# jason-huang03/SPH_Project

Hardware: AMD Instinct MI355X
Metric: particle-updates/sec (higher is better)
Workload: dtype f32

## Files before the change

### sph_project_amd/csrc/sph_device.hpp

```cpp
#pragma once
#include "sph_common.hpp"
#include <limits.h>

#ifndef SPH_FAST
#define SPH_FAST 0
#endif

__device__ __forceinline__ float fdiv(float a, float b) {
#if SPH_FAST
    return a * __builtin_amdgcn_rcpf(b);
#else
    return a / b;
#endif
}
__device__ __forceinline__ float fdiv2(float a, float b, float c) {
#if SPH_FAST
    return a * __builtin_amdgcn_rcpf(b * c);
#else
    return (a / b) / c;
#endif
}
__device__ __forceinline__ float fsqrt(float a) {
#if SPH_FAST
    return __builtin_amdgcn_sqrtf(a);
// ... 676 lines not shown
            const unsigned by = (cy > 0 ? 1u : 0u) | 2u | (cy < c.ny - 1 ? 4u : 0u);
            my_dom = (cx > 0 ? by : 0u) | (by << 3) | (cx < c.nx - 1 ? by << 6 : 0u);
        }
    }
    (&s_cnt[0][0])[tid] = 0;
    if (blk_flag) {
        const int anyf = __syncthreads_or((i < n && META_ACTIVE_FLUID(meta_i)) ? 1 : 0);
        if (tid == 0) blk_flag[blockIdx.x] = anyf ? 1 : 0;
    }
    unsigned long long peers = ~0ull;
#pragma unroll
    for (int bit = 0; bit < 6; ++bit) {
        const bool on = (key >> bit) & 1;
        const unsigned long long bal = __ballot(on);
        peers &= on ? bal : ~bal;
    }
    const unsigned long long below = (1ull << lane) - 1ull;
    const int rank_in_wave = __popcll(peers & below);
    __syncthreads();
    if (cellw && i < n) {
        const int e0 = (my_lin - s_c[0]) + my_dz0 + 1;
        cellw[i] = (unsigned)(e0 & 0xff) | ((unsigned)(my_dz + 1) << 8) | (my_dom << 11);
    }
    if ((peers & below) == 0ull) s_cnt[w][key] = __popcll(peers);
    if (tid < 9) {
        const int cfirst = s_c[0], clast = s_c[1];
        const int shift = (tid / 3 - 1) * c.ny * c.nz + (tid % 3 - 1) * c.nz;
        int lo = cfirst + shift - 1, hi = clast + shift + 1;
        int rs = 0, re = 0;
        if (clast >= cfirst && hi >= 0 && lo <= c.G - 1) {
            lo = lo < 0 ? 0 : lo;
            hi = hi > c.G - 1 ? c.G - 1 : hi;
            rs = cell_start[lo];
            re = cell_start[hi + 1];
        }
        int *h = blk_hdr + (size_t)blockIdx.x * BLK_HDR_INTS;
        if (tid == 0) { h[0] = cfirst; h[1] = clast; }
        h[2 + tid] = rs;
        h[11 + tid] = re - rs;
    }
    __syncthreads();
    if (perm) {
        const int tot = s_cnt[0][lane] + s_cnt[1][lane] + s_cnt[2][lane] + s_cnt[3][lane];
        const int incl = wave_incl_scan(tot);
        int dest = __shfl(incl - tot, key, 64) + rank_in_wave;
        for (int k = 0; k < w; ++k) dest += s_cnt[k][key];
        perm[i0 + dest] = (unsigned char)tid;
    }
}

__global__ void __launch_bounds__(256)
k_block_prep(const Consts c, const float4 *__restrict__ posv, const int *__restrict__ meta,
             const int *__restrict__ cell_start, int *__restrict__ blk_hdr, unsigned char *__restrict__ perm,
             int *__restrict__ blk_flag, const int *__restrict__ xidx, BlockPrepTables tabs, TilePlanOut plan, unsigned *__restrict__ cellw) {
    __shared__ int s_cnt[4][64];
    __shared__ int s_c[2];
    const int tid = threadIdx.x;
    const int i0 = blockIdx.x * 256;
    const int i = i0 + tid;
    const int n = live_n(c);
    if (plan.list_b && tid == 64 && i0 < n) {
        const int layer = c.ny * c.nz;
        const int r1 = plan.lo_layers > 0 ? cell_start[(plan.lo_layers < c.nx ? plan.lo_layers : c.nx) * layer] : 0;
        const int r2 = plan.hi_layers > 0 ? cell_start[(c.nx - plan.hi_layers > 0 ? c.nx - plan.hi_layers : 0) * layer] : n;
        const int nt = (n + 255) >> 8;
        int t1 = (r1 + 255) >> 8, t2 = r2 >> 8;
        if (t2 > nt) t2 = nt;
        if (t2 < t1) t2 = t1 = nt;
        const int t = (int)blockIdx.x, ni = t2 - t1;
        if (t < t1) plan.list_b[t] = t;
        else if (t >= t2) plan.list_b[t1 + (t - t2)] = t;
        else plan.list_i[t - t1] = t1 + xcd_remap(t - t1, ni);
        plan.cls[t] = (t < t1 || t >= t2) ? 1 : 0;
        if (t == 0) {
            plan.cnt[0] = nt - ni; plan.cnt[1] = ni;
            if (nt - ni > plan.bound_b && plan.status) atomicOr(plan.status, SLAB_ST_BOUND);
            if (plan.mirror_nb) *plan.mirror_nb = nt - ni;
        }
    }
    if (i0 >= n) {
        if (blk_flag && tid == 0) blk_flag[blockIdx.x] = 0;
        return;
    }
    float4 p = make_float4(0.f, 0.f, 0.f, 0.f);
    int meta_i = 0;
    if (i < n) {
        if (xidx) {
            const int x = xidx[i];
            const int kind = (int)(((unsigned)x) >> 28);
            if (kind >= 1 && kind <= 8) tabs.tab[kind - 1][x & 0x0fffffff] = i;
        }
        p = posv[i];
        if (blk_flag) meta_i = meta[i];
    }
    block_prep_tile(c, n, p, meta_i, cell_start, blk_hdr, perm, blk_flag, cellw, s_cnt, s_c);
}

__global__ void __launch_bounds__(256)
k_gather_prep(const Consts c, int n, const int *__restrict__ inv, SortArrays a, const int *__restrict__ cell_start,
              int *__restrict__ blk_hdr, unsigned char *__restrict__ perm, int *__restrict__ blk_flag, unsigned *__restrict__ cellw) {
    __shared__ int s_cnt[4][64];
    __shared__ int s_c[2];
    const int d = blockIdx.x * 256 + threadIdx.x;
    float4 p = make_float4(0.f, 0.f, 0.f, 0.f);
    int meta_i = 0;
    if (d < n) {
        const int i = inv[d];
        p = a.posv_in[i];
        meta_i = a.meta_in[i];
        a.posv_out[d] = p;
        a.velm_out[d] = a.velm_in[i];
        a.meta_out[d] = meta_i;
        a.pid_out[d] = a.pid_in[i];
        if (a.color_in) a.color_out[d] = a.color_in[i];
        if (a.rho_in) a.rho_out[d] = a.rho_in[i];
        if (a.orig_in) a.orig_out[d] = a.orig_in[i];
    }
    block_prep_tile(c, n, p, meta_i, cell_start, blk_hdr, perm, blk_flag, cellw, s_cnt, s_c);
}

__global__ void __launch_bounds__(256)
k_color_from_home(int n, const int *__restrict__ pid, const unsigned *__restrict__ home, unsigned *__restrict__ color) {
    const int i = blockIdx.x * 256 + threadIdx.x;
    if (i < n) color[i] = home[pid[i]];
}

__global__ void __launch_bounds__(256)
k_compact_blocks(const int *__restrict__ flag, int nb, int *__restrict__ list, int *__restrict__ count, volatile int *count_host) {
    __shared__ int s_w[4];
    const int per = (nb + 255) / 256;
    const int lo = threadIdx.x * per, hi = lo + per < nb ? lo + per : nb;
    int mine = 0;
    for (int b = lo; b < hi; ++b) mine += flag[b] ? 1 : 0;
    int tot;
    int at = block_excl_scan_256(mine, s_w, tot);
    for (int b = lo; b < hi; ++b) if (flag[b]) list[at++] = b;
    if (threadIdx.x == 0) { *count = tot; if (count_host) *count_host = tot; }
}

constexpr int SPH_NBR_LIGHT_CAP = 1280;
constexpr int SPH_NBR_HEAVY_BUDGET = 40960;
constexpr int SPH_NBR_MEDIUM_BYTES = 28;
constexpr int SPH_HEAVY_SB = 3;
constexpr int SPH_MEDIUM_SB = 3;
template <class P> constexpr int pass_slot_bytes() {
    return 16 + (P::HAS_B ? (int)sizeof(typename P::BT) : 0) + (PassC<P>::value ? (int)sizeof(typename PassC<P>::type) : 0);
}
template <class P, class = void> struct PassMediumOk { static constexpr bool value = false; };
template <class P> struct PassMediumOk<P, decltype((void)P::MEDIUM_OK)> { static constexpr bool value = P::MEDIUM_OK; };
template <class P> constexpr bool pass_is_medium() {
    return SPH_FAST && P::HAS_B && !pass_builds_masks<P>() &&
           (pass_slot_bytes<P>() <= SPH_NBR_MEDIUM_BYTES || (PassMediumOk<P>::value && pass_slot_bytes<P>() <= 32));
}
template <class P> constexpr int nbr_tile_cap() {
    const int per_slot = pass_slot_bytes<P>();
    const int budget = pass_is_medium<P>() ? 32768 : SPH_NBR_HEAVY_BUDGET;
    const int slots = (budget - 9 * NBR_CS_PITCH * 2 - 1536) / per_slot - NBR_PAD;
    return slots > SPH_NBR_LIGHT_CAP ? SPH_NBR_LIGHT_CAP : slots / 8 * 8;
}
__device__ __forceinline__ int run_of(int grouping, int g, int q) {
    const int i = g * 3 + q;
    return grouping ? (int)((0x861543720ull >> (4 * i)) & 15ull) : i;
}

template <int CAP>
__device__ __forceinline__ void nbr_plan(const int *__restrict__ hdr, int g, int qa, int fg, int (&rs_)[3], int (&ln_)[3], int (&lo_)[3],
                                         int &total, int &qb, unsigned &rm, bool &overflow, int grouping) {
    total = 0; qb = 3; rm = 7u; overflow = false;
#pragma unroll
    for (int q = 0; q < 3; ++q) {
        const int k = run_of(grouping, g, q);
        rs_[q] = hdr[2 + k];
        ln_[q] = hdr[11 + k] > 0 ? hdr[11 + k] : 0;
    }
    const int ulen = rs_[2] + ln_[2] - rs_[0];
    const bool chain = !grouping && ln_[0] > 0 && ln_[1] > 0 && ln_[2] > 0 && rs_[1] >= rs_[0] && rs_[1] <= rs_[0] + ln_[0] &&
                       rs_[2] >= rs_[1] && rs_[2] <= rs_[1] + ln_[1] && ulen >= ln_[2];
    if (qa == 0 && chain && ulen <= CAP && fg != 1 && fg != 5) {
        lo_[0] = lo_[1] = lo_[2] = -rs_[0];
        total = ulen;
    } else if (qa == 0 && ln_[0] + ln_[1] + ln_[2] <= CAP && fg != 1) {
        lo_[0] = -rs_[0]; lo_[1] = ln_[0] - rs_[1]; lo_[2] = ln_[0] + ln_[1] - rs_[2];
        total = ln_[0] + ln_[1] + ln_[2];
    } else {
        rm = 0u; qb = qa;
#pragma unroll
        for (int q = 0; q < 3; ++q) {
            lo_[q] = INT_MIN;
            if (q >= qa && q == qb && !overflow) {
                if (fg != 1 && total + ln_[q] <= CAP) { lo_[q] = total - rs_[q]; total += ln_[q]; qb = q + 1; rm |= 1u << q; }
                else if (q == qa) { overflow = true; qb = q + 1; rm |= 1u << q; }
            }
        }
    }
}
#ifdef SPH_TIMELINE
#define NBR_STAMP(k) do { if (timeline && threadIdx.x == 0) timeline[(size_t)blockIdx.x * 16 + (k)] = __builtin_readcyclecounter(); } while (0)
#else
#define NBR_STAMP(k) do { } while (0)
#endif
template <class P, int MASKMODE> constexpr int nbr_lds_bytes() {
    return (nbr_tile_cap<P>() + ((MASKMODE == 2 || pass_reuses_masks<P>()) ? 0 : NBR_PAD)) * (16 + (P::HAS_B ? (int)sizeof(typename P::BT) : 0) + (PassC<P>::value ? (int)sizeof(typename PassC<P>::type) : 0)) + 9 * NBR_CS_PITCH * 2 + 64;
}
constexpr int SPH_NBR_WAVES_LIGHT = SPH_FAST ? 6 : 4;
constexpr int SPH_NBR_WAVES_HEAVY = SPH_FAST ? 4 : 3;
template <class P, class = void> struct PassMaxWaves { static constexpr int value = 8; };
template <class P> struct PassMaxWaves<P, decltype((void)P::MAX_WAVES)> { static constexpr int value = P::MAX_WAVES; };
template <class P, int MASKMODE> constexpr int nbr_waves_per_simd() {
    const int w = P::HAS_B ? (pass_is_medium<P>() ? 5 : SPH_NBR_WAVES_HEAVY) : (sizeof(typename P::Own) <= 8 ? SPH_NBR_WAVES_LIGHT : 4);
    return w < PassMaxWaves<P>::value ? w : PassMaxWaves<P>::value;
}
__device__ __forceinline__ int split_lo(int ny, int y) { return ny == 3 ? y : (y == 0 ? 0 : 2); }
__device__ __forceinline__ int split_hi(int ny, int y) { return ny == 3 ? y + 1 : (y == 0 ? 2 : 3); }
template <class P, int MASKMODE>
__global__ void __launch_bounds__(P::BLOCK, (nbr_waves_per_simd<P, MASKMODE>()))
k_nbr_pass(const Consts c, const int *__restrict__ cell_start, const P p, DevScalars *__restrict__ scal,
           int nblocks, unsigned *__restrict__ nbr_mask, unsigned *__restrict__ nbr_mask_hi, int mask_stride,
           const int *__restrict__ blk_hdr, const unsigned char *__restrict__ lane_perm,
           unsigned long long *__restrict__ timeline, const int *__restrict__ stop_flag,
           const int *__restrict__ blk_list, const int *__restrict__ blk_count, const unsigned char *__restrict__ tile_skip) {
    const int stop_now = stop_flag ? *stop_flag : 0;
    const int list_len = blk_list ? *blk_count : INT_MAX;
    const int b_listed = blk_list ? blk_list[blockIdx.x] : 0;
    if (stop_now) return;
    if ((int)blockIdx.x >= list_len) {
        if constexpr (PassPrologue<P>::value) { if (blockIdx.x == 0 && blockIdx.y == 0) p.prologue(scal); }
        return;
    }
    constexpr int BLOCK = P::BLOCK;
    constexpr int CAP = nbr_tile_cap<P>();
    constexpr int NS = (CAP + BLOCK - 1) / BLOCK;
    constexpr int GROUPS = 3, RPG = 3;
    static_assert(P::GROUPS == 3 && BLOCK == 256, "lane permutation is stored as one byte per particle");
    typedef typename P::Own Own;
    typedef typename P::BT BT;
    constexpr int PAD = (MASKMODE == 2 || pass_reuses_masks<P>()) ? 0 : NBR_PAD;
    __shared__ float2 sT[2 * (CAP + PAD)];
    float2 *const sXY = sT;
    float2 *const sZW = sT + (CAP + PAD);
    constexpr int ZW_OFF = (CAP + PAD) * 8;
    __shared__ BT sB[P::HAS_B ? CAP + PAD : 1];
    __shared__ typename PassC<P>::type sC[PassC<P>::value ? CAP + PAD : 1];
    __shared__ unsigned short s_cs[9][NBR_CS_PITCH];
    __shared__ int s_loff[9];

    const int tid = threadIdx.x;
    NBR_STAMP(0);
    const int b = blk_list ? b_listed : xcd_remap(blockIdx.x, nblocks, c.xcd_chunk);
    const int i0 = b * BLOCK;
    const int who_early = lane_perm ? (int)lane_perm[i0 + tid] : tid;
    const int *hdr = blk_hdr + (size_t)b * BLK_HDR_INTS;
    const int cfirst = hdr[0], clast = hdr[1];
    const int skip_tile = tile_skip ? (int)tile_skip[b] : 0;
    const int n_live = live_n(c);
    if constexpr (PassWrench<P>::value) wrench_init_all(p.pose);
    if constexpr (PassPrologue<P>::value) { if (!p.prologue(scal)) return; }
    if (i0 >= n_live) {
        if constexpr (P::HAS_REDUCE) {
            if (tid == 0) {
                const int bs = red_slot(blk_list, b);
                if constexpr (PassSplit<P>::value) {
                    if (gridDim.y > 1) {
                        if (float *o = p.split_out(split_lo((int)gridDim.y, (int)blockIdx.y))) o[bs] = 0.0f;
                        if (gridDim.y == 2 && blockIdx.y == 0) { if (float *o = p.split_out(1)) o[bs] = 0.0f; }
                    } else p.red_out[bs] = 0.0f;
                }
                else p.red_out[bs] = 0.0f;
            }
        }
        return;
    }
    const int who = who_early;
    const int i = i0 + who;
    const bool valid = i < n_live;

    const int span = clast - cfirst;
    bool cs_lds = span >= 0 && span <= NBR_CS_SPAN;
#pragma unroll
    for (int k = 0; k < 9; ++k) cs_lds = cs_lds && hdr[11 + k] < 65536;
    const int ic = valid ? i : i0;
    const unsigned cw = reinterpret_cast<const unsigned *>(blk_hdr + (size_t)((mask_stride + 255) >> 8) * BLK_HDR_INTS)[ic];
    const float4 pi = p.posv[ic];
    Own own;
    bool active = p.begin(c, ic, pi, own) && valid;
    unsigned mk0[3] = {0u, 0u, 0u};
    if (MASKMODE == 2 && pass_mask_pipe<P>()) {
        const int g0 = (PassSplit<P>::value && gridDim.y > 1) ? split_lo((int)gridDim.y, (int)blockIdx.y) : 0;
#pragma unroll
        for (int q = 0; q < 3; ++q) mk0[q] = nbr_mask[(size_t)run_of(c.run_grouping, g0, q) * mask_stride + i];
    }
    typedef typename PassC<P>::type CT;
    const int g_first = (PassSplit<P>::value && gridDim.y > 1) ? split_lo((int)gridDim.y, (int)blockIdx.y) : 0;
    (void)g_first;
    if (cs_lds && tid < NBR_CS_PITCH) {
        const int tc = tid < span + 4 ? tid : span + 3;
        int cs_[9];
#pragma unroll
        for (int k = 0; k < 9; ++k) {
            int cell = cfirst + (k / 3 - 1) * c.ny * c.nz + (k % 3 - 1) * c.nz - 1 + tc;
            cell = cell < 0 ? 0 : (cell > c.G ? c.G : cell);
            cs_[k] = cell_start[cell];
        }
        if (tid < span + 4) {
#pragma unroll
            for (int k = 0; k < 9; ++k) s_cs[k][tid] = (unsigned short)(cs_[k] - hdr[2 + k]);
        }
    }
    const int e0 = (int)(cw & 0xffu);
    const int e1 = e0 + (int)((cw >> 8) & 7u);
    const unsigned dom = cw >> 11;
    if (skip_tile) return;
    if (__syncthreads_or(active ? 1 : 0)) {
        NBR_STAMP(1);
        unsigned npairs = 0;
        const bool is_split = PassSplit<P>::value && gridDim.y > 1;
        const int g_lo = is_split ? split_lo((int)gridDim.y, (int)blockIdx.y) : 0;
        const int g_hi = is_split ? split_hi((int)gridDim.y, (int)blockIdx.y) : GROUPS;
        unsigned mkn[RPG] = {mk0[0], mk0[1], mk0[2]};
#pragma unroll 1
        for (int g = g_lo, qa = 0; g < (c.force_global == 11 ? 0 : g_hi); ) {
            int rs_[RPG], ln_[RPG], lo_[RPG];
            int total, qb;
            unsigned rm;
            bool overflow;
            nbr_plan<CAP>(hdr, g, qa, c.force_global, rs_, ln_, lo_, total, qb, rm, overflow, c.run_grouping);
#define NBR_IN_ROUND(q) ((rm >> (q)) & 1u)
            if (tid < RPG) {
                s_loff[g * RPG + tid] = tid == 0 ? lo_[0] : (tid == 1 ? lo_[1] : lo_[2]);
                if (overflow && tid == qa && (tid == 0 ? ln_[0] : (tid == 1 ? ln_[1] : ln_[2])) > 0) atomicAdd(&scal->fallback[c.stat_bank][b & (SPH_STAT_SLOTS - 1)], 1ull);
            }
            unsigned mk[RPG], mh[RPG] = {0u, 0u, 0u};
            if constexpr (pass_mask_pipe<P>() || MASKMODE != 2) {
#pragma unroll
                for (int q = 0; q < RPG; ++q) mk[q] = mkn[q];
            } else {
#pragma unroll
                for (int q = 0; q < RPG; ++q) mk[q] = nbr_mask[(size_t)run_of(c.run_grouping, g, q) * mask_stride + i];
            }
            constexpr int SB = pass_is_medium<P>() ? (NS > SPH_MEDIUM_SB ? SPH_MEDIUM_SB : NS)
                                                   : ((P::HAS_B && sizeof(BT) >= 16) ? ((PassUsesJ0<P>::value || !SPH_FAST) ? 2 : (SPH_HEAVY_SB < NS ? SPH_HEAVY_SB : NS)) : NS);
            const int n0 = lo_[0] != INT_MIN ? ln_[0] : 0;
            const int n01 = n0 + (lo_[1] != INT_MIN ? ln_[1] : 0);
            const bool stage_now = total > 0 && c.force_global != 10;
            float4 a_[SB];
            BT b_[SB];
            CT c_[SB];
            if (stage_now) {
#pragma unroll
                for (int u = 0; u < SB; ++u) {
                    int t = tid + u * BLOCK;
                    t = t < total ? t : total - 1;
                    const int j = t < n0 ? t - lo_[0] : (t < n01 ? t - lo_[1] : t - lo_[2]);
                    a_[u] = pass_stage(p, c, j, b_[u], c_[u]);
                }
            }
            if (MASKMODE == 2 && pass_mask_pipe<P>()) {
                const int gn = qb >= RPG ? (g + 1 < GROUPS ? g + 1 : g) : g;
#pragma unroll
                for (int q = 0; q < RPG; ++q) mkn[q] = nbr_mask[(size_t)run_of(c.run_grouping, gn, q) * mask_stride + i];
            }
            bool inr[RPG];
            int js_[RPG], m_[RPG];
            bool wide = false, longrun = false;
#pragma unroll
            for (int q = 0; q < RPG; ++q) {
                const int k = run_of(c.run_grouping, g, q);
                inr[q] = NBR_IN_ROUND(q) && active && ((dom >> k) & 1u);
                js_[q] = 0; m_[q] = 0;
                if (inr[q]) {
                    if (cs_lds) {
                        const int o0 = lds_ld_u16(&s_cs[k][e0]);
                        js_[q] = rs_[q] + o0;
                        m_[q] = lds_ld_u16(&s_cs[k][e1]) - o0;
                    } else {
                        float px = pi.x, py = pi.y, pz = pi.z;
                        asm volatile("" : "+v"(px), "+v"(py), "+v"(pz));
                        const int xx = cell_coord_x(c, px) + k / 3 - 1, yy = cell_coord(py, c.grid_size, c.ny) + k % 3 - 1;
                        const int cz = cell_coord_z(c, pz);
                        const int z0 = cz > 0 ? cz - 1 : 0;
                        const int z1 = cz < c.nz - 1 ? cz + 1 : c.nz - 1;
                        const int lin0 = (xx * c.ny + yy) * c.nz + z0;
                        js_[q] = cell_start[lin0];
                        m_[q] = cell_start[lin0 + (z1 - z0) + 1] - js_[q];
                    }
                    wide = wide || m_[q] > 32;
                    longrun = longrun || m_[q] > 64;
                }
                if (MASKMODE == 2 && m_[q] > 32 && c.force_global != 12) mh[q] = nbr_mask_hi[(size_t)k * mask_stride + i];
                if (MASKMODE == 2 && (m_[q] <= 0 || c.force_global == 12)) mk[q] = 0u;
            }
            if (stage_now) {
#pragma unroll
                for (int u = 0; u < SB; ++u) {
                    const int t = tid + u * BLOCK;
                    if (t < total) {
                        sXY[t] = make_float2(a_[u].x, a_[u].y);
                        sZW[t] = make_float2(a_[u].z, a_[u].w);
                        if (P::HAS_B) sB[t] = b_[u];
                        if (PassC<P>::value) sC[t] = c_[u];
                    }
                }
            }
#pragma unroll 1
            for (int u0 = SB; u0 < NS && u0 * BLOCK < total && stage_now; u0 += SB) {
#pragma unroll
                for (int u = 0; u < SB; ++u) {
                    const int t = tid + (u0 + u) * BLOCK;
                    if (t < total) {
                        const int j = t < n0 ? t - lo_[0] : (t < n01 ? t - lo_[1] : t - lo_[2]);
                        a_[u] = pass_stage(p, c, j, b_[u], c_[u]);
                    }
                }
#pragma unroll
                for (int u = 0; u < SB; ++u) {
                    const int t = tid + (u0 + u) * BLOCK;
                    if (t < total) {
                        sXY[t] = make_float2(a_[u].x, a_[u].y);
                        sZW[t] = make_float2(a_[u].z, a_[u].w);
                        if (P::HAS_B) sB[t] = b_[u];
                        if (PassC<P>::value) sC[t] = c_[u];
                    }
                }
            }
            __syncthreads();
            NBR_STAMP(2 + g * 4);
            if (overflow) {
                const int k = run_of(c.run_grouping, g, qa);
                const int rsq = qa == 0 ? rs_[0] : (qa == 1 ? rs_[1] : rs_[2]);
                const int lnq = qa == 0 ? ln_[0] : (qa == 1 ? ln_[1] : ln_[2]);
                const bool in = qa == 0 ? inr[0] : (qa == 1 ? inr[1] : inr[2]);
                const int js = in ? (qa == 0 ? js_[0] : (qa == 1 ? js_[1] : js_[2])) : 0;
                const int m = in ? (qa == 0 ? m_[0] : (qa == 1 ? m_[1] : m_[2])) : 0;
                unsigned long long w01 = 0ull;
#pragma unroll 1
                for (int cs0 = 0; cs0 < lnq; cs0 += CAP) {
                    const int cl = lnq - cs0 < CAP ? lnq - cs0 : CAP;
                    for (int t = tid; t < cl; t += BLOCK) {
                        BT bj; CT cj;
                        const float4 a = pass_stage(p, c, rsq + cs0 + t, bj, cj);
                        sXY[t] = make_float2(a.x, a.y);
                        sZW[t] = make_float2(a.z, a.w);
                        if (P::HAS_B) sB[t] = bj;
                        if (PassC<P>::value) sC[t] = cj;
                    }
                    __syncthreads();
                    process_chunk<ZW_OFF, MASKMODE>(c, p, own, i, pi.x, pi.y, pi.z, js, js + m, rsq + cs0, rsq + cs0 + cl, sXY, sZW, sB, sC, npairs, w01);
                    __syncthreads();
                }
                if (MASKMODE == 1 && in) {
                    nbr_mask[(size_t)k * mask_stride + i] = (unsigned)w01;
                    if (m > 32) nbr_mask_hi[(size_t)k * mask_stride + i] = (unsigned)(w01 >> 32);
                }
            } else if (c.force_global == 4 || __any(longrun)) {
#pragma unroll 1
                for (int q = 0; q < RPG; ++q) {
                    const int k = run_of(c.run_grouping, g, q);
                    const bool in = q == 0 ? inr[0] : (q == 1 ? inr[1] : inr[2]);
                    const int js = in ? (q == 0 ? js_[0] : (q == 1 ? js_[1] : js_[2])) : 0;
                    const int m = in ? (q == 0 ? m_[0] : (q == 1 ? m_[1] : m_[2])) : 0;
                    const int loff = q == 0 ? lo_[0] : (q == 1 ? lo_[1] : lo_[2]);
                    const int cs = loff == INT_MIN ? 0 : -loff;
                    const int ce = loff == INT_MIN ? 0 : cs + total;
                    unsigned long long w01 = 0ull;
                    process_chunk<ZW_OFF, MASKMODE>(c, p, own, i, pi.x, pi.y, pi.z, js, js + m, cs, ce, sXY, sZW, sB, sC, npairs, w01);
                    if (MASKMODE == 1 && in) {
                        nbr_mask[(size_t)k * mask_stride + i] = (unsigned)w01;
                        if (m > 32) nbr_mask_hi[(size_t)k * mask_stride + i] = (unsigned)(w01 >> 32);
                    }
                }
            } else {
                const bool anywide = __any(wide);
                unsigned ab[RPG];
#pragma unroll
                for (int q = 0; q < RPG; ++q) {
                    const int k = run_of(c.run_grouping, g, q);
                    const int base = inr[q] ? js_[q] + lo_[q] : 0;
                    unsigned nm, nh = 0u;
                    if (MASKMODE == 2) {
                        nm = mk[q]; nh = mh[q];
                    } else {
                        const int mlo = m_[q] < 32 ? m_[q] : 32;
                        constexpr bool LEAN1 = pass_reuses_masks<P>();
                        nm = c.force_global == 13 ? 0u : phase1_mask<ZW_OFF, LEAN1>(sXY, base, mlo, pi.x, pi.y, pi.z, c.h2);
                        if (anywide) nh = phase1_mask<ZW_OFF, LEAN1>(sXY, m_[q] > 32 ? base + 32 : 0, m_[q] > 32 ? m_[q] - 32 : 0, pi.x, pi.y, pi.z, c.h2);
                        const unsigned self = (unsigned)(i - js_[q]);
                        if (self < 32u) nm &= ~(1u << self);
                        else if (self < 64u) nh &= ~(1u << (self - 32u));
                        if (MASKMODE == 1 && inr[q]) {
                            nbr_mask[(size_t)k * mask_stride + i] = nm;
                            if (m_[q] > 32) nbr_mask_hi[(size_t)k * mask_stride + i] = nh;
                        }
                    }
// ... 113 lines not shown
```

### sph_project_amd/csrc/sph_passes.hpp

```cpp
#pragma once
#include "sph_device.hpp"

typedef float WrenchRows[4][SPH_NOBJ][6];
__device__ __forceinline__ WrenchRows &wrench_rows() {
    __shared__ WrenchRows s_rows;
    return s_rows;
}
typedef float WrenchCom[SPH_NOBJ][3];
__device__ __forceinline__ WrenchCom &wrench_com() {
    __shared__ WrenchCom s_com;
    return s_com;
}
__device__ __forceinline__ void wrench_init_all(const RigidPose *pose) {
    float *r = &wrench_rows()[0][0][0];
    for (int k = threadIdx.x; k < 4 * SPH_NOBJ * 6; k += 256) r[k] = 0.0f;
    if (threadIdx.x < SPH_NOBJ * 3) (&wrench_com()[0][0])[threadIdx.x] = (&pose->com[0][0])[threadIdx.x];
}
__device__ __forceinline__ void wrench_flush_all(DevScalars *scal) {
    const int k = threadIdx.x;
    if (k >= SPH_NOBJ * 6) return;
    const WrenchRows &w = wrench_rows();
    const int obj = k / 6, q = k % 6;
    const float v = ((w[0][obj][q] + w[1][obj][q]) + w[2][obj][q]) + w[3][obj][q];
    if (v != 0.0f)
// ... 210 lines not shown
                const int obj = (int)(-bj.w) - 2;
                const float fx = fdiv(-acx * o.m, c.rho0), fy = fdiv(-acy * o.m, c.rho0), fz = fdiv(-acz * o.m, c.rho0);
                const float rx = a.x - wrench_com()[obj][0], ry = a.y - wrench_com()[obj][1], rz = a.z - wrench_com()[obj][2];
                add_wrench(scal, obj, fx, fy, fz, ry * fz - rz * fy, rz * fx - rx * fz, rx * fy - ry * fx);
            }
        }
#else
        const float rn2 = g.rn * g.rn;
        float gx, gy, gz;
        if (AF || bj.w >= 0.0f) {
            const float cst = o.st_m * a.w;
            const float w = r2 > c.diameter2 ? K::W(c, g) : K::Wd(c);
            o.sx -= (cst * dx) * w; o.sy -= (cst * dy) * w; o.sz -= (cst * dz) * w;
            if (skip_viscosity) return;
            K::grad(c, dx, dy, dz, g, gx, gy, gz);
            const float v_xy = (o.vx - bj.x) * dx + (o.vy - bj.y) * dy + (o.vz - bj.z) * dz;
            const float m_ij = (o.m + a.w) * 0.5f;
            const float cc = fdiv2(c.cv * m_ij, bj.w, rn2 + c.visc_eps) * v_xy;
            o.ax += cc * gx; o.ay += cc * gy; o.az += cc * gz;
        } else {
            if (skip_viscosity) return;
            K::grad(c, dx, dy, dz, g, gx, gy, gz);
            const float v_xy = (o.vx - bj.x) * dx + (o.vy - bj.y) * dy + (o.vz - bj.z) * dz;
            const float cc = fdiv2(c.cvb * a.w, o.rho, rn2 + c.visc_eps) * v_xy;
            const float acx = cc * gx, acy = cc * gy, acz = cc * gz;
            o.ax += acx; o.ay += acy; o.az += acz;
            if (bj.w <= -2.0f) {
                const int obj = (int)(-bj.w) - 2;
                const float fx = fdiv(-acx * o.m, c.rho0), fy = fdiv(-acy * o.m, c.rho0), fz = fdiv(-acz * o.m, c.rho0);
                const float rx = a.x - wrench_com()[obj][0], ry = a.y - wrench_com()[obj][1], rz = a.z - wrench_com()[obj][2];
                add_wrench(scal, obj, fx, fy, fz, ry * fz - rz * fy, rz * fx - rx * fz, rx * fy - ry * fx);
            }
        }
#endif
    }
    __device__ float finish(const Consts &c, int i, const float4 &, Own &o) const {
        float ax = c.gx, ay = c.gy, az = c.gz;
        ax += o.sx; ay += o.sy; az += o.sz;
        ax += fdiv(o.ax, c.rho0); ay += fdiv(o.ay, c.rho0); az += fdiv(o.az, c.rho0);
        if (acc_out) acc_out[i] = make_float4(ax, ay, az, 0.0f);
        float vx = o.vx, vy = o.vy, vz = o.vz;
        if (visc_vel) { const float4 v = velm[i]; vx = v.x; vy = v.y; vz = v.z; }
        vel_out[i] = make_float4(vx + c.dt * ax, vy + c.dt * ay, vz + c.dt * az, o.m);
        return 0.0f;
    }
    __device__ void passive(const Consts &, int i, const float4 &) const { vel_out[i] = velm[i]; }
};

__device__ __forceinline__ void enforce_boundary(const Consts &c, float &x, float &y, float &z, float &vx,
                                                 float &vy, float &vz) {
    float nx = 0.f, ny = 0.f, nz = 0.f;
    const float ox = x, oy = y, oz = z;
    if (ox > c.hix) { nx += 1.0f; x = c.hix; }
    if (ox <= c.pad) { nx += -1.0f; x = c.pad; }
    if (oy > c.hiy) { ny += 1.0f; y = c.hiy; }
    if (oy <= c.pad) { ny += -1.0f; y = c.pad; }
    if (oz > c.hiz) { nz += 1.0f; z = c.hiz; }
    if (oz <= c.pad) { nz += -1.0f; z = c.pad; }
    const float len = __builtin_sqrtf(nx * nx + ny * ny + nz * nz);
    if (len > 1e-6f) {
        const float ux = nx / len, uy = ny / len, uz = nz / len;
        const float s = (1.0f + 0.5f) * (vx * ux + vy * uy + vz * uz);
        vx -= s * ux; vy -= s * uy; vz -= s * uz;
    }
}

template <bool AF>
struct PressurePass {
    static constexpr bool HAS_WRENCH = !AF;
    static constexpr int BLOCK = 256, GROUPS = 3;
    static constexpr bool USES_J = !AF;
    static constexpr bool HAS_B = true, COUNT_PAIRS = true;
    static constexpr int PAIR_WEIGHT = 1;
    static constexpr bool HAS_REDUCE = false;
    typedef float BT;
    struct Own { float pt, p, rho2, ax, ay, az, x, y, z, m0; };
    const float4 *posv; const int *meta; const float *ptm, *prs, *rho;
    float4 *velm;
    float4 *acc, *posv_out; DevScalars *scal; const RigidPose *pose; float rho0;
    int integrate;

    __device__ float4 stage_impl(int j, BT &bj) const {
        const float4 p = posv[j];
        const float m = velm[j].w;
        if (AF) { bj = ptm[j]; return make_float4(p.x, p.y, p.z, m); }
        const int mt = meta[j];
        const bool fl = META_MAT(mt) == 1;
        bj = fl ? ptm[j] : (META_DYN(mt) ? -2.0f - (float)META_OBJ(mt) : -1.0f);
        return make_float4(p.x, p.y, p.z, fl ? m : rho0 * p.w);
    }
    __device__ float4 loadA(int j) const { BT b; return stage_impl(j, b); }
    __device__ BT loadB(int j) const { BT b; stage_impl(j, b); return b; }
    __device__ float4 stage(const Consts &, int j, BT &bj) const { return stage_impl(j, bj); }
    __device__ bool begin(const Consts &c, int i, const float4 &pi, Own &o) const {
        bool ok = true;
        if (!AF) { const int m = meta[i]; ok = META_ACTIVE_FLUID(m) && META_DYN(m); }
        else if (c.ghosts) ok = !META_GHOST(meta[i]);
        o.x = pi.x; o.y = pi.y; o.z = pi.z; o.m0 = rho0 * pi.w;
        o.pt = ptm[i]; o.p = prs[i];
        const float r = rho[i];
        o.rho2 = r * r;
        o.ax = o.ay = o.az = 0.0f;
        return ok;
    }
    __device__ void pair(const Consts &c, Own &o, float dx, float dy, float dz, float r2, const float4 &a,
                         const BT &bj, int j) const {
        const Geom g = geom(c, r2);
#if SPH_FAST
        if (AF || bj >= 0.0f) {
            const float k = (-a.w * (o.pt + bj)) * kernGradScale(c, g);
            o.ax += k * dx; o.ay += k * dy; o.az += k * dz;
            return;
        }
#endif
        float gx, gy, gz;
        kernGrad(c, dx, dy, dz, g, gx, gy, gz);
        if (AF || bj >= 0.0f) {
            const float cc = -a.w * (o.pt + bj);
            o.ax += cc * gx; o.ay += cc * gy; o.az += cc * gz;
        } else {
            const float cc = fdiv(-a.w * o.p, o.rho2);
            o.ax += cc * gx; o.ay += cc * gy; o.az += cc * gz;
            if (bj <= -2.0f) {
                const int obj = (int)(-bj) - 2;
                const float cf = fdiv(a.w * o.p, o.rho2);
                const float fx = (cf * gx) * o.m0, fy = (cf * gy) * o.m0, fz = (cf * gz) * o.m0;
                const float rx = o.x - wrench_com()[obj][0], ry = o.y - wrench_com()[obj][1], rz = o.z - wrench_com()[obj][2];
                add_wrench(scal, obj, fx, fy, fz, ry * fz - rz * fy, rz * fx - rx * fz, rx * fy - ry * fx);
            }
        }
    }
    __device__ float finish(const Consts &c, int i, const float4 &pi, Own &o) const {
        acc[i] = make_float4(o.ax, o.ay, o.az, 0.0f);
        if (!integrate) return 0.0f;
        const float4 v = velm[i];
        float vx = v.x + c.dt * o.ax, vy = v.y + c.dt * o.ay, vz = v.z + c.dt * o.az;
        float x = pi.x + c.dt * vx, y = pi.y + c.dt * vy, z = pi.z + c.dt * vz;
        enforce_boundary(c, x, y, z, vx, vy, vz);
        posv_out[i] = make_float4(x, y, z, pi.w);
        velm[i] = make_float4(vx, vy, vz, v.w);
        return 0.0f;
    }
    __device__ void passive(const Consts &, int i, const float4 &pi) const {
        acc[i] = make_float4(0.f, 0.f, 0.f, 0.f);
        if (integrate) posv_out[i] = pi;
    }
};

template <bool AF, bool UM = false, bool CNT = false>
struct WcsphForcePass {
    static constexpr bool HAS_WRENCH = !AF;
    static constexpr int BLOCK = 256, GROUPS = 3;
    static constexpr bool USES_J = !AF;
    static constexpr bool HAS_B = true, HAS_C = true;
    static constexpr bool COUNT_PAIRS = CNT;
    static constexpr int MAX_WAVES = CNT ? (SPH_FAST ? 4 : 3) : 8;
    static constexpr bool MASK_PIPELINE = AF;
    static constexpr int PAIR_WEIGHT = 3;
    static constexpr bool HAS_REDUCE = false;
    typedef float4 BT;
    typedef float CT;
    struct Own {
        float vx, vy, vz, m, rho, st_m, sx, sy, sz, ax, ay, az;
        float pt, p, rho2, px, py, pz, x, y, z, m0;
        float cvm, cstm;
        int dyn;
        int lin_new;
    };
    static constexpr bool NEXT_HASH = AF;
    const float4 *posv, *velm; const int *meta; const float *rho_raw, *ptm, *prs, *rho;
    float4 *vel_out, *acc, *posv_out; DevScalars *scal; const RigidPose *pose; float rho0;
    HaloSend hs;
    NextHash nh;
    __device__ int cell_of(const Consts &c, float x, float y, float z) const {
        return (cell_coord_x(c, x) * c.ny + cell_coord(y, c.grid_size, c.ny)) * c.nz + cell_coord_z(c, z);
    }

    __device__ float4 loadA(int j) const { return posv[j]; }
    __device__ float4 stage(const Consts &, int j, BT &bj, CT &cj) const {
        const float4 p = ldg_idx(posv, j);
        const float4 v = ldg_idx(velm, j);
        if (AF) {
            bj = make_float4(v.x, v.y, v.z, ldg_idx(rho_raw, j));
            cj = ldg_idx(ptm, j);
            return make_float4(p.x, p.y, p.z, v.w);
        }
        const int m = meta[j];
        const bool fl = META_MAT(m) == 1;
        bj = make_float4(v.x, v.y, v.z, fl ? rho_raw[j] : (META_DYN(m) ? -2.0f - (float)META_OBJ(m) : -1.0f));
        cj = fl ? ptm[j] : 0.0f;
        return make_float4(p.x, p.y, p.z, fl ? v.w : rho0 * p.w);
    }
    __device__ bool begin(const Consts &c, int i, const float4 &pi, Own &o) const {
        o.dyn = 1;
        bool ok = true;
        if (AF && c.ghosts) ok = !META_GHOST(meta[i]);
        if (!AF) {
            const int m = meta[i];
            ok = META_ACTIVE_FLUID(m);
            if (!ok) return false;
            o.dyn = META_DYN(m);
        }
        const float4 v = velm[i];
        o.vx = v.x; o.vy = v.y; o.vz = v.z; o.m = v.w;
        o.rho = rho_raw[i];
#if SPH_FAST
        o.st_m = (fdiv(c.st, v.w) * c.rho0) * c.kW;
#else
        o.st_m = fdiv(c.st, v.w);
#endif
        o.cvm = c.cv * ((v.w + v.w) * 0.5f); o.cstm = o.st_m * v.w;
        o.sx = o.sy = o.sz = 0.0f;
        o.ax = o.ay = o.az = 0.0f;
        o.x = pi.x; o.y = pi.y; o.z = pi.z; o.m0 = rho0 * pi.w;
        o.pt = ptm[i]; o.p = prs[i];
        const float r = rho[i];
        o.rho2 = r * r;
        o.px = o.py = o.pz = 0.0f;
        return ok;
    }
    __device__ void pair(const Consts &c, Own &o, float dx, float dy, float dz, float r2, const float4 &a,
                         const BT &bj, const CT &cj, int j) const {
        const Geom g = geom(c, r2);
#if SPH_FAST
        const float gs = kernGradScale(c, g);
        const float v_xy = (o.vx - bj.x) * dx + (o.vy - bj.y) * dy + (o.vz - bj.z) * dz;
        if (AF || bj.w >= 0.0f) {
            const float w = r2 > c.diameter2 ? kernWpoly(g) : c.Wd_poly;
            const float cw = (UM ? o.cstm : o.st_m * a.w) * w;
            const float cvm = UM ? o.cvm : c.cv * ((o.m + a.w) * 0.5f);
            const float cc = fdiv2(cvm, bj.w, r2 + c.visc_eps) * v_xy;
            const float k = cc * gs - cw;
            o.ax += k * dx; o.ay += k * dy; o.az += k * dz;
            const float cp = (-(UM ? o.m : a.w) * (o.pt + cj)) * gs;
            o.px += cp * dx; o.py += cp * dy; o.pz += cp * dz;
        } else {
            const float k = (fdiv2(c.cvb * a.w, o.rho, r2 + c.visc_eps) * v_xy) * gs;
            const float acx = k * dx, acy = k * dy, acz = k * dz;
            o.ax += acx; o.ay += acy; o.az += acz;
            const float cp = fdiv(-a.w * o.p, o.rho2) * gs;
            o.px += cp * dx; o.py += cp * dy; o.pz += cp * dz;
            if (bj.w <= -2.0f) {
                const int obj = (int)(-bj.w) - 2;
                float fx = fdiv(-acx * o.m, c.rho0), fy = fdiv(-acy * o.m, c.rho0), fz = fdiv(-acz * o.m, c.rho0);
                float rx = a.x - wrench_com()[obj][0], ry = a.y - wrench_com()[obj][1], rz = a.z - wrench_com()[obj][2];
                float tx = ry * fz - rz * fy, ty = rz * fx - rx * fz, tz = rx * fy - ry * fx;
                if (AF || o.dyn) {
                    const float cf = -cp * o.m0;
                    const float gxf = cf * dx, gyf = cf * dy, gzf = cf * dz;
                    rx = o.x - wrench_com()[obj][0]; ry = o.y - wrench_com()[obj][1]; rz = o.z - wrench_com()[obj][2];
                    tx += ry * gzf - rz * gyf; ty += rz * gxf - rx * gzf; tz += rx * gyf - ry * gxf;
                    fx += gxf; fy += gyf; fz += gzf;
                }
                add_wrench(scal, obj, fx, fy, fz, tx, ty, tz);
            }
        }
#else
        const float rn2 = g.rn * g.rn;
        float gx, gy, gz;
        kernGrad(c, dx, dy, dz, g, gx, gy, gz);
        const float v_xy = (o.vx - bj.x) * dx + (o.vy - bj.y) * dy + (o.vz - bj.z) * dz;
        if (AF || bj.w >= 0.0f) {
            const float cst = o.st_m * a.w;
            const float w = r2 > c.diameter2 ? kernW(c, g) : c.Wd;
            o.sx -= (cst * dx) * w; o.sy -= (cst * dy) * w; o.sz -= (cst * dz) * w;
            const float m_ij = (o.m + a.w) * 0.5f;
            const float cc = fdiv2(c.cv * m_ij, bj.w, rn2 + c.visc_eps) * v_xy;
            o.ax += cc * gx; o.ay += cc * gy; o.az += cc * gz;
            const float cp = -a.w * (o.pt + cj);
            o.px += cp * gx; o.py += cp * gy; o.pz += cp * gz;
        } else {
            const float cc = fdiv2(c.cvb * a.w, o.rho, rn2 + c.visc_eps) * v_xy;
            const float acx = cc * gx, acy = cc * gy, acz = cc * gz;
            o.ax += acx; o.ay += acy; o.az += acz;
            const float cp = fdiv(-a.w * o.p, o.rho2);
            o.px += cp * gx; o.py += cp * gy; o.pz += cp * gz;
            if (bj.w <= -2.0f) {
                const int obj = (int)(-bj.w) - 2;
                float fx = fdiv(-acx * o.m, c.rho0), fy = fdiv(-acy * o.m, c.rho0), fz = fdiv(-acz * o.m, c.rho0);
                float rx = a.x - wrench_com()[obj][0], ry = a.y - wrench_com()[obj][1], rz = a.z - wrench_com()[obj][2];
                float tx = ry * fz - rz * fy, ty = rz * fx - rx * fz, tz = rx * fy - ry * fx;
                if (AF || o.dyn) {
                    const float cf = fdiv(a.w * o.p, o.rho2);
                    const float gxf = (cf * gx) * o.m0, gyf = (cf * gy) * o.m0, gzf = (cf * gz) * o.m0;
                    rx = o.x - wrench_com()[obj][0]; ry = o.y - wrench_com()[obj][1]; rz = o.z - wrench_com()[obj][2];
                    tx += ry * gzf - rz * gyf; ty += rz * gxf - rx * gzf; tz += rx * gyf - ry * gxf;
                    fx += gxf; fy += gyf; fz += gzf;
                }
                add_wrench(scal, obj, fx, fy, fz, tx, ty, tz);
            }
        }
#endif
    }
    __device__ float finish(const Consts &c, int i, const float4 &pi, Own &o) const {
        float ax = c.gx, ay = c.gy, az = c.gz;
        ax += o.sx; ay += o.sy; az += o.sz;
        ax += fdiv(o.ax, c.rho0); ay += fdiv(o.ay, c.rho0); az += fdiv(o.az, c.rho0);
        float vx = o.vx + c.dt * ax, vy = o.vy + c.dt * ay, vz = o.vz + c.dt * az;
        if (!AF && !o.dyn) {
            vel_out[i] = make_float4(vx, vy, vz, o.m);
            acc[i] = make_float4(0.f, 0.f, 0.f, 0.f);
            posv_out[i] = pi;
            if (hs.on) halo_presend(c, hs, i, pi, make_float4(vx, vy, vz, o.m), rho[i]);
            if (NEXT_HASH && nh.on) o.lin_new = cell_of(c, pi.x, pi.y, pi.z);
            return 0.0f;
        }
        acc[i] = make_float4(o.px, o.py, o.pz, 0.0f);
        vx = vx + c.dt * o.px; vy = vy + c.dt * o.py; vz = vz + c.dt * o.pz;
        float x = pi.x + c.dt * vx, y = pi.y + c.dt * vy, z = pi.z + c.dt * vz;
        enforce_boundary(c, x, y, z, vx, vy, vz);
        posv_out[i] = make_float4(x, y, z, pi.w);
        vel_out[i] = make_float4(vx, vy, vz, o.m);
        if (hs.on) halo_presend(c, hs, i, make_float4(x, y, z, pi.w), make_float4(vx, vy, vz, o.m), rho[i]);
        if (NEXT_HASH && nh.on) o.lin_new = cell_of(c, x, y, z);
        return 0.0f;
    }
    __device__ void passive(const Consts &c, int i, const float4 &pi) const {
        const float4 v = velm[i];
        vel_out[i] = v;
        acc[i] = make_float4(0.f, 0.f, 0.f, 0.f);
        posv_out[i] = pi;
        if (hs.on) halo_presend(c, hs, i, pi, v, rho[i]);
    }
};

template <class K = CubicKernel>
struct RigidVolumePass {
    static constexpr int MODES = 0b001;
    static constexpr int MAX_WAVES = 5;
    static constexpr int BLOCK = 256, GROUPS = 3;
    static constexpr bool USES_J = false;
    static constexpr bool HAS_B = false, COUNT_PAIRS = false;
    static constexpr int PAIR_WEIGHT = 0;
    static constexpr bool HAS_REDUCE = false;
    typedef int BT;
    struct Own { float sum; int obj; };
    float4 *posv; float4 *velm; const int *meta;

    __device__ float4 stage_impl(int j) const {
        const float4 p = posv[j];
        const int m = meta[j];
        const int key = META_MAT(m) == 2 ? META_OBJ(m) : -100;
        return make_float4(p.x, p.y, p.z, __int_as_float(key));
    }
    __device__ float4 loadA(int j) const { return stage_impl(j); }
    __device__ BT loadB(int) const { return 0; }
    __device__ float4 stage(const Consts &, int j, BT &) const { return stage_impl(j); }
    __device__ bool begin(const Consts &c, int i, const float4 &pi, Own &o) const {
        const int m = meta[i];
        if (META_MAT(m) != 2 || META_GHOST(m) || META_FRESH(m) || !(up_coord(c, pi) <= c.g_upper)) return false;
        o.obj = META_OBJ(m);
        o.sum = K::W0(c);
        return true;
    }
    __device__ void pair(const Consts &c, Own &o, float, float, float, float r2, const float4 &a, const BT &,
                         int) const {
        if (__float_as_int(a.w) == o.obj) o.sum += K::W(c, geom(c, r2));
    }
    __device__ float finish(const Consts &c, int i, const float4 &pi, Own &o) const {
        const float V = 1.0f / o.sum;
        posv[i] = make_float4(pi.x, pi.y, pi.z, V);
        float4 v = velm[i];
        v.w = c.rho0 * V;
        velm[i] = v;
        return 0.0f;
    }
    __device__ void passive(const Consts &, int, const float4 &) const {}
};
```

Baseline: 4.914 billion.

## Pack candidate pressure term into staged float4 to fit five workgroups per CU

For the fast, all-fluid, uniform-mass force pass, the separate per-candidate scalar array is dropped and the scalar is stored in the w lane of the staged position float4. This is safe because with uniform mass the mass comes from the owner instead. The smaller LDS slot lets the tile budget drop to 32 KB, so five waves per SIMD can be requested, with a staging depth of two. Per-particle uniform values are forced into scalar registers with readfirstlane. The costs are a smaller neighbour tile and a reliance on mass really being uniform across the wave.

New measurement: 5.118 billion, median of 6. 4.1% higher.

```diff
diff --git a/sph_project_amd/csrc/sph_device.hpp b/sph_project_amd/csrc/sph_device.hpp
--- a/sph_project_amd/csrc/sph_device.hpp
+++ b/sph_project_amd/csrc/sph_device.hpp
@@ -852,10 +852,16 @@
     return SPH_FAST && P::HAS_B && !pass_builds_masks<P>() &&
            (pass_slot_bytes<P>() <= SPH_NBR_MEDIUM_BYTES || (PassMediumOk<P>::value && pass_slot_bytes<P>() <= 32));
 }
+template <class P, class = void> struct PassFiveWg { static constexpr bool value = false; };
+template <class P> struct PassFiveWg<P, decltype((void)P::FIVE_WG)> { static constexpr bool value = P::FIVE_WG; };
+constexpr int SPH_FIVE_WG_SB = 2;
+constexpr int SPH_LDS_GRANULE = 1280;
 template <class P> constexpr int nbr_tile_cap() {
     const int per_slot = pass_slot_bytes<P>();
-    const int budget = pass_is_medium<P>() ? 32768 : SPH_NBR_HEAVY_BUDGET;
-    const int slots = (budget - 9 * NBR_CS_PITCH * 2 - 1536) / per_slot - NBR_PAD;
+    const int budget = (pass_is_medium<P>() || PassFiveWg<P>::value) ? 32768 : SPH_NBR_HEAVY_BUDGET;
+    const int pad = (PassFiveWg<P>::value && pass_reuses_masks<P>()) ? 0 : NBR_PAD;
+    const int reserve = PassFiveWg<P>::value ? SPH_LDS_GRANULE : 1536;
+    const int slots = (budget - 9 * NBR_CS_PITCH * 2 - reserve) / per_slot - pad;
     return slots > SPH_NBR_LIGHT_CAP ? SPH_NBR_LIGHT_CAP : slots / 8 * 8;
 }
 __device__ __forceinline__ int run_of(int grouping, int g, int q) {
@@ -907,7 +913,7 @@
 template <class P, class = void> struct PassMaxWaves { static constexpr int value = 8; };
 template <class P> struct PassMaxWaves<P, decltype((void)P::MAX_WAVES)> { static constexpr int value = P::MAX_WAVES; };
 template <class P, int MASKMODE> constexpr int nbr_waves_per_simd() {
-    const int w = P::HAS_B ? (pass_is_medium<P>() ? 5 : SPH_NBR_WAVES_HEAVY) : (sizeof(typename P::Own) <= 8 ? SPH_NBR_WAVES_LIGHT : 4);
+    const int w = P::HAS_B ? ((pass_is_medium<P>() || PassFiveWg<P>::value) ? 5 : SPH_NBR_WAVES_HEAVY) : (sizeof(typename P::Own) <= 8 ? SPH_NBR_WAVES_LIGHT : 4);
     return w < PassMaxWaves<P>::value ? w : PassMaxWaves<P>::value;
 }
 __device__ __forceinline__ int split_lo(int ny, int y) { return ny == 3 ? y : (y == 0 ? 0 : 2); }
@@ -1037,7 +1043,7 @@
 #pragma unroll
                 for (int q = 0; q < RPG; ++q) mk[q] = nbr_mask[(size_t)run_of(c.run_grouping, g, q) * mask_stride + i];
             }
-            constexpr int SB = pass_is_medium<P>() ? (NS > SPH_MEDIUM_SB ? SPH_MEDIUM_SB : NS)
+            constexpr int SB = pass_is_medium<P>() ? (NS > SPH_MEDIUM_SB ? SPH_MEDIUM_SB : NS) : PassFiveWg<P>::value ? SPH_FIVE_WG_SB
                                                    : ((P::HAS_B && sizeof(BT) >= 16) ? ((PassUsesJ0<P>::value || !SPH_FAST) ? 2 : (SPH_HEAVY_SB < NS ? SPH_HEAVY_SB : NS)) : NS);
             const int n0 = lo_[0] != INT_MIN ? ln_[0] : 0;
             const int n01 = n0 + (lo_[1] != INT_MIN ? ln_[1] : 0);
diff --git a/sph_project_amd/csrc/sph_passes.hpp b/sph_project_amd/csrc/sph_passes.hpp
--- a/sph_project_amd/csrc/sph_passes.hpp
+++ b/sph_project_amd/csrc/sph_passes.hpp
@@ -386,12 +386,14 @@
     static constexpr bool HAS_WRENCH = !AF;
     static constexpr int BLOCK = 256, GROUPS = 3;
     static constexpr bool USES_J = !AF;
-    static constexpr bool HAS_B = true, HAS_C = true;
+    static constexpr bool HAS_B = true;
     static constexpr bool COUNT_PAIRS = CNT;
     static constexpr int MAX_WAVES = CNT ? (SPH_FAST ? 4 : 3) : 8;
     static constexpr bool MASK_PIPELINE = AF;
     static constexpr int PAIR_WEIGHT = 3;
     static constexpr bool HAS_REDUCE = false;
+    static constexpr bool FIVE_WG = SPH_FAST && AF && UM && !CNT;
+    static constexpr bool HAS_C = !FIVE_WG;
     typedef float4 BT;
     typedef float CT;
     struct Own {
@@ -425,6 +427,11 @@
         cj = fl ? ptm[j] : 0.0f;
         return make_float4(p.x, p.y, p.z, fl ? v.w : rho0 * p.w);
     }
+    __device__ float4 stage(const Consts &c, int j, BT &bj) const {
+        CT cj;
+        const float4 a = stage(c, j, bj, cj);
+        return make_float4(a.x, a.y, a.z, cj);
+    }
     __device__ bool begin(const Consts &c, int i, const float4 &pi, Own &o) const {
         o.dyn = 1;
         bool ok = true;
@@ -444,6 +451,11 @@
         o.st_m = fdiv(c.st, v.w);
 #endif
         o.cvm = c.cv * ((v.w + v.w) * 0.5f); o.cstm = o.st_m * v.w;
+        if (FIVE_WG) {
+            o.m = __int_as_float(__builtin_amdgcn_readfirstlane(__float_as_int(o.m)));
+            o.cvm = __int_as_float(__builtin_amdgcn_readfirstlane(__float_as_int(o.cvm)));
+            o.cstm = __int_as_float(__builtin_amdgcn_readfirstlane(__float_as_int(o.cstm)));
+        }
         o.sx = o.sy = o.sz = 0.0f;
         o.ax = o.ay = o.az = 0.0f;
         o.x = pi.x; o.y = pi.y; o.z = pi.z; o.m0 = rho0 * pi.w;
@@ -526,6 +538,10 @@
         }
 #endif
     }
+    __device__ void pair(const Consts &c, Own &o, float dx, float dy, float dz, float r2, const float4 &a, const BT &bj, int j) const {
+        static_assert(FIVE_WG, "A.w is the candidate's mass everywhere else");
+        pair(c, o, dx, dy, dz, r2, a, bj, a.w, j);
+    }
     __device__ float finish(const Consts &c, int i, const float4 &pi, Own &o) const {
         float ax = c.gx, ay = c.gy, az = c.gz;
         ax += o.sx; ay += o.sy; az += o.sz;
```
